# simonhmartin/genomics_general

Measured on AMD Instinct MI355X. Metric: windows_per_sec, higher is better.
Workload: dtype u32 bit-planes / int32 counts / f64 statistics

## Files before the change

genomics_general_amd/csrc/pg_internal.h:

```cpp
#pragma once
#include <hip/hip_runtime.h>
#include <stdint.h>
#include "../../include/popgen_hip.h"
#include "pg_nib.h"

#define PG_MAX_POPS 16
#define PG_SITES_PER_BLOCK 1024
#define PG_ABBA_SITES_PER_BLOCK 4096
#define PG_ABBA_NSUM 6
#define PG_FOURPOP_NSUM 14
#define PG_XV_PLANES 2

#define PG_GROUP 64
#define PG_GROUP_MAX 128
#define PG_XV_CAP(grp) (3 * (grp))
#define PG_XV_CAP_DEFAULT(grp) ((grp) + 1)
#define PG_NP_MAX_SITES 256
#define PG_FLAG_MISMATCH 1
#define PG_FLAG_XV_OVERFLOW 2
#define PG_FLAG_FUSE_STALL 4

struct PgTask2 {
    int32_t row0, nsub, col0, lower;
};

struct PgSynthParams {
    uint64_t seed;
    int64_t first_site_index, scaf_len;
    int32_t n_dip, n_pops, var_thr, miss_thr;
};


void pg_launch_nib_pack(hipStream_t st, const int8_t *src, int S, int n_hap, int64_t n_rows, int8_t *gt, int RS);
void pg_launch_nib_expand(hipStream_t st, const int8_t *gt, int RS, int64_t n_rows, int8_t *dst, int S);
void pg_launch_synth(hipStream_t st, int8_t *gt, int RS, int n_hap, int64_t site0, int64_t n_sites,
                     const int32_t *slot_gen_hap, PgSynthParams p);

void pg_launch_popdist_fin(hipStream_t st, const int32_t *Cmat, const int32_t *Dmat, int N, int cN, int cshift, int n_win,
                           const int32_t *pop_start, int n_pops, int min_pair_sites, double *sum_out,
                           int64_t *cnt_out, int all_diploid, const int64_t *win_lo = nullptr, const int64_t *win_hi = nullptr,
                           long long skip_upto = -1);

void pg_launch_popdist_np(hipStream_t st, const int32_t *Cmat, const int32_t *Dmat, int N, int cN, int cshift, int n_win,
                          const int32_t *pop_start, int n_pops, const int32_t *ref_row, const int32_t *pop_rank,
                          const int32_t *task_tree, const int32_t *trees, int max_leaves, int max_side, int min_pair_sites,
                          double min_data, int do_pairs, double *sums, int64_t *cnts, double *out, const int64_t *win_lo,
                          const int64_t *win_hi, long long max_sites);

void pg_launch_indpair_fin(hipStream_t st, const int32_t *Cmat, const int32_t *Dmat, int N, int cN, int cshift, int n_win,
                           const int32_t *samp_start, const int32_t *samp_rank, int n_samp, int min_pair_sites, double *sum_out,
                           int64_t *cnt_out, int mean_mode);


void pg_launch_abba(hipStream_t st, const int8_t *gt, int RS, const int64_t *win_lo, const int64_t *win_hi,
                    int n_win, int max_chunks, const int32_t *pop_start, int p1, int p2, int p3, int p4,
                    double min_data, int sel, int nsum, double *part_sums, int64_t *part_used, double *sums_out,
                    int64_t *used_out, uint32_t *flags, int64_t base, long long max_sites);

void pg_launch_popfreq(hipStream_t st, const int8_t *gt, int RS, int n_hap, const int64_t *win_lo,
                       const int64_t *win_hi, int n_win, int max_chunks, const int32_t *pop_start, int n_pops,
                       unsigned long long *l_out, unsigned long long *S_out, unsigned long long *pairsum_out,
                       uint32_t *flags, int64_t base);
void pg_launch_popfreq_ordered(hipStream_t st, const int8_t *gt, int RS, const int64_t *win_lo, const int64_t *win_hi, int n_win,
                               const int32_t *pop_start, int n_pops, const uint32_t *flags, int64_t base, double *theta_out);

void pg_launch_site_counts(hipStream_t st, const int8_t *gt, int RS, int64_t site_lo, int64_t site_hi,
                           const int32_t *pop_start, int n_pops, int32_t *cnt_out);
void pg_launch_site_target(hipStream_t st, const int32_t *cnt, int64_t n_sites, int n_pops, int target, double min_data, int as_counts,
                           int has_threshold, double threshold, double *f_out, long long *i_out, uint8_t *keep_out);

void pg_launch_hap_called(hipStream_t st, const int8_t *gt, int RS, int n_hap, const int64_t *win_lo,
                          const int64_t *win_hi, int n_win, int max_chunks, unsigned long long *out);

void pg_launch_pack2(hipStream_t st, const int8_t *gt, int RS, const int64_t *win_lo, const int64_t *win_hi,
                     const int64_t *goff, const int64_t *vgoff, int n_win, int max_groups, int64_t total_groups, uint32_t *Vp,
                     int NPv, uint32_t *XV, int NP, int32_t *nw, int dip, int32_t *mismatch, uint32_t *pres, int capg, int grp);
bool pg_pack_needs_presence(int NP);
struct PgFuseArgs {
    int32_t n_win, kparts, n_units, T, diag;
    int32_t *Cmat;
    signed char a[8][4], b[8][2];
    unsigned char mask[8];
};
bool pg_pack_fuse_fits(int NP, int NPv, int n_units, int n_win);
int pg_launch_pack_fused(hipStream_t st, const int8_t *gt, int RS, const int64_t *win_lo, const int64_t *win_hi, const int64_t *goff,
                         int n_win, int64_t max_words, int64_t avg_words, uint32_t *XV, int NP, int32_t *nw, int dip, int32_t *mismatch,
                         int capg, int n_units, int32_t *Cmat);
void pg_launch_expand(hipStream_t st, const int32_t *Cmat, const int32_t *Dmat, int N, int cN, int cshift, int n_win,
                      int32_t *Cfull, int32_t *Dfull);
void pg_launch_pairC(hipStream_t st, const uint32_t *Vp, const int64_t *vgoff, int n_win, const PgTask2 *tasks, int n_tasks,
                     int NPv, int n_units, int diag, int64_t avg_wq, int32_t *Cmat);
void pg_launch_pairD(hipStream_t st, const uint32_t *XY, const int32_t *nw, const int64_t *goff, int n_win,
                     const PgTask2 *tasks, int n_tasks, int NP, int N, int64_t avg_groups, int32_t *Dmat, int capg);
void pg_launch_pairC_mfma(hipStream_t st, const uint32_t *Vp, const int64_t *vgoff, int n_win, int NPv, int n_units, int diag,
                          int64_t avg_wq, int64_t max_sites, int32_t *Cmat);
void pg_launch_pairD_mfma(hipStream_t st, const uint32_t *XV, const int32_t *nw, const int64_t *goff, int n_win, int NP, int N,
                          int64_t avg_words, int64_t max_vsites, int32_t *Dmat, int capg);

bool pg_pair_tile_fits(int NPv);
int pg_launch_pairC_tile(hipStream_t st, const uint32_t *Vp, const int64_t *vgoff, int n_win, int NPv, int n_units, int diag,
                         int64_t avg_wq, int64_t max_sites, int32_t *Cmat);

bool pg_pair_big_fits(int NPv, int n_units);
void pg_launch_pairC_big(hipStream_t st, const uint32_t *Vp, const int64_t *vgoff, int n_win, int NPv, int n_units, int diag,
                         int64_t avg_wq, int64_t max_sites, int32_t *Cmat);

void pg_launch_sample_het(hipStream_t st, const int32_t *Cmat, const int32_t *Dmat, int N, int cN, int cshift, int n_win,
                          const int32_t *samp_start, int n_samp, int min_pair_sites, double *out);
void pg_launch_hapstats(hipStream_t st, const int32_t *Cmat, const int32_t *Dmat, int N, int cN, int cshift, int n_win,
                        const int32_t *pop_start, int n_pops, int max_pop, const int32_t *order, int min_pair_sites, int diag_nan,
                        double max_dist, uint32_t *bits, size_t bits_per_window, double *out);
void pg_launch_unpack(hipStream_t st, const uint8_t *cells, int n_cols, int64_t n_rows, const int32_t *slot_src, int n_hap,
                      int8_t *gt, int RS);
void pg_launch_flag_export(hipStream_t st, int32_t *flag, double *dst);
void pg_launch_popstats(hipStream_t st, const double *sums, const int64_t *cnts, int n_win, const int32_t *pop_start,
                        int n_pops, double min_data, int do_pairs, double *out, const int64_t *win_lo = nullptr,
                        const int64_t *win_hi = nullptr, long long skip_upto = -1);
```

genomics_general_amd/csrc/pg_pair2.hip:

```cpp
#include "pg_internal.h"

#include <algorithm>
#include <cstdlib>
#include <cstring>

typedef __attribute__((address_space(4))) const uint32_t CU32;

__device__ __forceinline__ void store16(uint32_t *p, uint32_t a, uint32_t b, uint32_t c, uint32_t d) {
    *reinterpret_cast<uint4 *>(p) = make_uint4(a, b, c, d);
}

__device__ __forceinline__ void btrans4(uint32_t t0, uint32_t t1, uint32_t t2, uint32_t t3, uint32_t r[4]) {
    const uint32_t lo01 = __builtin_amdgcn_perm(t1, t0, 0x05010400u), hi01 = __builtin_amdgcn_perm(t1, t0, 0x07030602u);
    const uint32_t lo23 = __builtin_amdgcn_perm(t3, t2, 0x05010400u), hi23 = __builtin_amdgcn_perm(t3, t2, 0x07030602u);
    r[0] = __builtin_amdgcn_perm(lo23, lo01, 0x05040100u);
    r[1] = __builtin_amdgcn_perm(lo23, lo01, 0x07060302u);
    r[2] = __builtin_amdgcn_perm(hi23, hi01, 0x05040100u);
    r[3] = __builtin_amdgcn_perm(hi23, hi01, 0x07060302u);
}

struct RowOff { int v[16]; };

__device__ __forceinline__ RowOff make_row_off(int RS) {
    RowOff ro;
// ... 383 lines not shown
        const uint32_t piece = (a >= q ? (o >> (a - q)) : (o << (q - a))) & (0x11111111u << q);
        pa[a] = q ? (pa[a] | piece) : piece;
    }
}

__device__ __forceinline__ void word_called_presence_keep(const uint32_t d[32], uint32_t v[8], uint32_t pa[4], uint32_t R[4][8]) {
#pragma unroll
    for (int q = 0; q < 4; ++q) {
        uint32_t re[4], ro[4];
        trans_even(d + 8 * q, re);
        trans_odd(d + 8 * q, ro);
        keep_presence(q, re, ro, R[q], pa);
#pragma unroll
        for (int k = 0; k < 8; ++k) {
            const uint32_t t = R[q][k] + 0x77777777u;
            const uint32_t c = (q == 3 ? t : (t >> (3 - q))) & (0x11111111u << q);
            v[k] = q ? (v[k] | c) : c;
        }
    }
}

template <int NWAVE, bool STAGED>
struct XvSink {
    XvWin win;
    int *sh_slot;
    uint4 *cell;
    int stride, burst;
    int nxs;

    __device__ __forceinline__ XvSink(const XvWin &w, int *sh_slot_, uint4 *cell_, int stride_, int burst_)
        : win(w), sh_slot(sh_slot_), cell(cell_), stride(stride_), burst(burst_), nxs(0) {}
    __device__ __forceinline__ void flush() {
        if (!nxs) return;
        const int slot0 = xv_reserve<NWAVE>(win.nwb, nxs, sh_slot);
        for (int k = 0; k < nxs; ++k)
            if (win.template holds<NWAVE>(slot0 + k)) {
                uint4 *o = reinterpret_cast<uint4 *>(win.word(slot0 + k));
#pragma unroll
                for (int i = 0; i < 4; ++i) o[i] = cell[(4 * k + i) * stride];
            }
        nxs = 0;
    }
    __device__ __forceinline__ void put(const uint32_t xo[8], const uint32_t vo[8]) {
        if (STAGED) {
            if (win.has_data) {
#pragma unroll
                for (int i = 0; i < 4; ++i) cell[(4 * nxs + i) * stride] = make_uint4(xo[2 * i], vo[2 * i], xo[2 * i + 1], vo[2 * i + 1]);
            }
            if (++nxs == burst) flush();
        } else {
            const int slot = xv_reserve<NWAVE>(win.nwb, 1, sh_slot);
            if (win.template holds<NWAVE>(slot)) {
                uint32_t *o = win.word(slot);
#pragma unroll
                for (int i = 0; i < 4; ++i) store16(o + 4 * i, xo[2 * i], vo[2 * i], xo[2 * i + 1], vo[2 * i + 1]);
            }
        }
    }
};

__device__ __forceinline__ uint32_t nz_nibbles(uint32_t x) { return ((x + 0x77777777u) >> 3) & 0x11111111u; }


template <class Sink>
struct VsCompactor {
    uint32_t cur[8], xo[8], vo[8];
    int cnt;
    uint32_t MA, ME;
    Sink &out;

    __device__ __forceinline__ explicit VsCompactor(Sink &s) : cnt(0), MA(0u), ME(0u), out(s) {
#pragma unroll
        for (int k = 0; k < 8; ++k) cur[k] = xo[k] = vo[k] = 0u;
    }
    __device__ __forceinline__ void finish_dword(int qd) {
        const uint32_t nME = ~ME;
#pragma unroll
        for (int k = 0; k < 8; ++k) {
            xo[k] |= nz_nibbles(cur[k] & MA) << qd;
            vo[k] |= nz_nibbles(cur[k] & nME) << qd;
            cur[k] = 0u;
        }
        MA = 0u;
        ME = 0u;
    }
    __device__ __forceinline__ void store_word() {
        out.put(xo, vo);
#pragma unroll
        for (int k = 0; k < 8; ++k) xo[k] = vo[k] = 0u;
    }
    __device__ __forceinline__ void append(const uint32_t (&Rq)[8], int j, uint32_t A, uint32_t E) {
        const int sh = 4 * (cnt & 7);
#pragma unroll
        for (int k = 0; k < 8; ++k) cur[k] |= __builtin_amdgcn_ubfe(Rq[k], 4 * j, 4) << sh;
        MA |= A << sh;
        ME |= E << sh;
        ++cnt;
        if ((cnt & 7) == 0) {
            finish_dword((cnt >> 3) - 1);
            if (cnt == 32) {
                store_word();
                cnt = 0;
            }
        }
    }
    __device__ __forceinline__ void finish() {
        if (cnt & 7) finish_dword(cnt >> 3);
        if (cnt) store_word();
    }
};

template <class Sink>
__device__ __forceinline__ void emit_poly_sites(const uint32_t pr[4], const uint32_t (&R)[4][8], VsCompactor<Sink> &vs, int lane) {
    const uint32_t m0 = poly_mask(pr);
    if (m0) {
        const int lb = lane & 31;
        const uint32_t Pl = __builtin_amdgcn_ubfe(pr[0], lb, 1) | (__builtin_amdgcn_ubfe(pr[1], lb, 1) << 1) |
                            (__builtin_amdgcn_ubfe(pr[2], lb, 1) << 2) | (__builtin_amdgcn_ubfe(pr[3], lb, 1) << 3);
        const uint32_t A0l = Pl & (0u - Pl);
#pragma unroll
        for (int q = 0; q < 4; ++q) {
            uint32_t mq = m0 & (0x11111111u << q);
            while (mq) {
                const int bit = __builtin_ctz(mq);
                mq &= mq - 1u;
                vs.append(R[q], bit >> 2, (uint32_t)__builtin_amdgcn_readlane((int)A0l, bit), 0u);
            }
        }
        const uint32_t m3 = tri_mask(pr);
        if (m3) {
#pragma unroll 1
            for (int pass = 1; pass < 3; ++pass) {
                uint32_t m = pass == 1 ? m3 : quad_mask(pr);
                while (m) {
                    const int bit = __builtin_ctz(m);
                    m &= m - 1u;
                    const uint32_t P = (uint32_t)__builtin_amdgcn_readlane((int)Pl, bit);
                    const uint32_t A0 = P & (0u - P), P1 = P ^ A0, A1 = P1 & (0u - P1), P2 = P1 ^ A1, A2 = P2 & (0u - P2);
                    const uint32_t A = pass == 1 ? A1 : A2;
                    const int q = bit & 3;
                    if (q == 0) vs.append(R[0], bit >> 2, A, (A - 1u) & P);
                    else if (q == 1) vs.append(R[1], bit >> 2, A, (A - 1u) & P);
                    else if (q == 2) vs.append(R[2], bit >> 2, A, (A - 1u) & P);
                    else vs.append(R[3], bit >> 2, A, (A - 1u) & P);
                }
            }
        }
    }
}

constexpr int PACK_FUSE_XC = 2;
constexpr int PACK_FUSE_NB = 3;
constexpr int PACK_FUSE_SPINS = 1 << 22;
typedef int fz_v8i __attribute__((ext_vector_type(8)));
typedef float fz_v16f __attribute__((ext_vector_type(16)));

__device__ __forceinline__ fz_v16f fz_mfma(const fz_v8i &a, const fz_v8i &b, const fz_v16f &c) {
    return __builtin_amdgcn_mfma_scale_f32_32x32x64_f8f6f4(a, b, c, 4, 4, 0, 0, 0, 0);
}

__device__ __forceinline__ void fuse_frags(const uint4 *fb, int s, int UW, const int ia[4], const int ib[2], fz_v8i fa_[4], fz_v8i fb_[2]) {
#pragma unroll
    for (int p = 0; p < 4; ++p) {
        const uint4 x = fb[2 * s * UW + ia[p]];
        fa_[p][0] = (int)x.x; fa_[p][1] = (int)x.y; fa_[p][2] = (int)x.z; fa_[p][3] = (int)x.w;
    }
#pragma unroll
    for (int p = 0; p < 2; ++p) {
        const uint4 x = fb[2 * s * UW + ib[p]];
        fb_[p][0] = (int)x.x; fb_[p][1] = (int)x.y; fb_[p][2] = (int)x.z; fb_[p][3] = (int)x.w;
    }
}

__device__ __forceinline__ bool fuse_win_decode(int per_win, int n_win, int &win, int &rem) {
    const int xcd = blockIdx.x & 7;
    const int v = blockIdx.x >> 3;
    const int full = n_win >> 3;
    if (v < full * per_win) {
        win = (v / per_win) * 8 + xcd;
        rem = v % per_win;
        return true;
    }
    const int total = (n_win & 7) * per_win, q = (total + 7) >> 3;
    const int vt = v - full * per_win, lin = xcd * q + vt;
    if (vt >= q || lin >= total) return false;
    win = full * 8 + lin / per_win;
    rem = lin % per_win;
    return true;
}

template <int DIP>
__device__ __forceinline__ void pack3_fused(const int8_t *__restrict__ gt, int RS, const int64_t *__restrict__ win_lo,
                                            const int64_t *__restrict__ win_hi, const int64_t *__restrict__ goff,
                                            uint32_t *__restrict__ XV, int NP, int32_t *__restrict__ nw,
                                            int32_t *__restrict__ mismatch, int capg, const PgFuseArgs &fa) {
    constexpr int VN = DIP ? 4 : 8;
    extern __shared__ uint4 fz_lds[];
    int b, kp;
    if (!fuse_win_decode(fa.kparts, fa.n_win, b, kp)) return;
    const int UW = 32 * fa.T;
    const int lane = threadIdx.x & 63, wave = __builtin_amdgcn_readfirstlane(threadIdx.x >> 6);
    uint4 *const frag = fz_lds;
    uint4 *const stage_x = fz_lds + PACK_FUSE_NB * 8 * UW + wave * (PACK_FUSE_XC * 4 * 64);
    int *const ready = reinterpret_cast<int *>(fz_lds + PACK_FUSE_NB * 8 * UW + 8 * (PACK_FUSE_XC * 4 * 64)), *const done = ready + PACK_FUSE_NB;
    const int64_t lo = win_lo[b], hi = win_hi[b];
    const int W = (int)((hi - lo + 31) >> 5);
    const int w_begin = (int)((long long)W * kp / fa.kparts), w_end = (int)((long long)W * (kp + 1) / fa.kparts);
    const int nit = (w_end - w_begin + 7) >> 3;
    const int h0 = 8 * lane;
    const bool has_data = h0 < 2 * RS;
    const int u0 = VN * lane;
    uint32_t bad = 0u;
    typedef XvSink<1, true> Sink;
    Sink xs(make_xv_win(XV, goff, b, capg, NP, h0, nw, mismatch, has_data), nullptr,  stage_x + lane,  64,
             PACK_FUSE_XC);
    VsCompactor<Sink> vs(xs);
    auto word_rsrc = [&](int w) -> __amdgpu_buffer_rsrc_t {
        const int64_t row = lo + 32ll * w;
        const int n = w < w_end ? (int)((hi - row) < 32 ? (hi - row) : 32) : 0;
        return group_rsrc(gt, RS, n ? row : lo, n);
    };
    const int r = lane & 31, kb = lane >> 5;
    int ia[4], ib[2];
#pragma unroll
    for (int p = 0; p < 4; ++p) ia[p] = kb * UW + 32 * (int)fa.a[wave][p] + r;
#pragma unroll
    for (int p = 0; p < 2; ++p) ib[p] = kb * UW + 32 * (int)fa.b[wave][p] + r;
    fz_v16f acc[4];
#pragma unroll
    for (int p = 0; p < 4; ++p)
#pragma unroll
        for (int e = 0; e < 16; ++e) acc[p][e] = 0.0f;
    if (threadIdx.x < 2 * PACK_FUSE_NB) ready[threadIdx.x] = threadIdx.x == 2 * PACK_FUSE_NB - 1 ? -8 : 0;
    for (int i = threadIdx.x; i < 8 * UW; i += 512) frag[(PACK_FUSE_NB - 1) * 8 * UW + i] = make_uint4(0u, 0u, 0u, 0u);
    bool stalled = false;
    auto wait_ge = [&](int *ctr, int target) {
        for (int spins = 0; __builtin_amdgcn_readfirstlane(__hip_atomic_load(ctr, __ATOMIC_ACQUIRE, __HIP_MEMORY_SCOPE_WORKGROUP)) < target;) {
            __builtin_amdgcn_s_sleep(1);
            if (++spins > PACK_FUSE_SPINS) { stalled = true; break; }
        }
    };
    auto arrive = [&](int *ctr) {
        if (lane == 0) __hip_atomic_fetch_add(ctr, 1, __ATOMIC_RELEASE, __HIP_MEMORY_SCOPE_WORKGROUP);
    };
    uint32_t dn[32];
#pragma unroll
    for (int s = 0; s < 32; ++s) dn[s] = 0u;
    const RowOff ro = make_row_off(RS);
    const int lane_off = has_data ? 4 * lane : 0x40000000;
    word_load(word_rsrc(w_begin + wave), lane_off, RS, 0, ro, dn);
    __syncthreads();
    int slot = 0, round8 = 0, pslot = PACK_FUSE_NB - 1, pround8 = -8;
    for (int it = 0; it < nit; ++it) {
        const int w = w_begin + 8 * it + wave;
        uint32_t pa[4] = {0u, 0u, 0u, 0u};
        uint32_t R[4][8];
        const bool live = w < w_end;
        uint32_t d[32];
#pragma unroll
        for (int s = 0; s < 32; ++s) d[s] = dn[s];
        word_load(word_rsrc(w + 8), lane_off, RS, 0, ro, dn);
        wait_ge(&ready[pslot], pround8 + 8);
        const uint4 *fb = frag + pslot * 8 * UW;
#pragma unroll
        for (int q = 0; q < 4; ++q) {
            fz_v8i fa_[4], fb_[2];
            fuse_frags(fb, q, UW, ia, ib, fa_, fb_);
            uint32_t re[4], rq[4];
            __builtin_amdgcn_sched_barrier(0);
            trans_even(d + 8 * q, re);
            asm volatile("" : "+v"(re[0]), "+v"(re[1]), "+v"(re[2]), "+v"(re[3]));
            __builtin_amdgcn_sched_barrier(0);
            acc[0] = fz_mfma(fa_[0], fb_[0], acc[0]);
            __builtin_amdgcn_sched_barrier(0);
            trans_odd(d + 8 * q, rq);
            asm volatile("" : "+v"(rq[0]), "+v"(rq[1]), "+v"(rq[2]), "+v"(rq[3]));
            __builtin_amdgcn_sched_barrier(0);
            acc[1] = fz_mfma(fa_[1], fb_[1], acc[1]);
            __builtin_amdgcn_sched_barrier(0);
            keep_presence(q, re, rq, R[q], pa);
            asm volatile("" : "+v"(pa[0]), "+v"(pa[1]), "+v"(pa[2]), "+v"(pa[3]));
            __builtin_amdgcn_sched_barrier(0);
            acc[2] = fz_mfma(fa_[2], fb_[0], acc[2]);
            acc[3] = fz_mfma(fa_[3], fb_[1], acc[3]);
            __builtin_amdgcn_sched_barrier(0);
        }
        arrive(&done[pslot]);
        wait_ge(&done[slot], round8);
        {
            uint4 *cell = frag + (slot * 8 + wave) * UW + u0;
#pragma unroll
            for (int k = 0; k < VN; ++k) {
                const int hk = DIP ? 2 * k : k;
                uint32_t c[4];
#pragma unroll
                for (int q = 0; q < 4; ++q) {
                    const uint32_t t = R[q][hk] + 0x77777777u;
                    if (DIP) bad |= t ^ (R[q][hk + 1] + 0x77777777u);
                    c[q] = (t >> 3) & 0x11111111u;
                }
                if (u0 + k < UW) cell[k] = make_uint4(c[0], c[1], c[2], c[3]);
            }
        }
        arrive(&ready[slot]);
        if (live) {
            uint32_t pr[4];
#pragma unroll
            for (int a = 0; a < 4; ++a) pr[a] = pa[a];
            wave_or4(pr);
            emit_poly_sites(pr, R, vs, lane);
        }
        pslot = slot;
        pround8 = round8;
        if (++slot == PACK_FUSE_NB) { slot = 0; round8 += 8; }
    }
    wait_ge(&ready[pslot], pround8 + 8);
#pragma unroll
    for (int q = 0; q < 4; ++q) {
        fz_v8i fa_[4], fb_[2];
        fuse_frags(frag + pslot * 8 * UW, q, UW, ia, ib, fa_, fb_);
#pragma unroll
        for (int p = 0; p < 4; ++p) acc[p] = fz_mfma(fa_[p], fb_[p & 1], acc[p]);
    }
    if (stalled && lane == 0) atomicOr(mismatch, PG_FLAG_FUSE_STALL);
    vs.finish();
    xs.flush();
    if (DIP && (bad & 0x88888888u)) atomicOr(mismatch, 1);
    const int n = fa.n_units, atomic = fa.kparts > 1;
    int32_t *Cw = fa.Cmat + (size_t)b * n * n;
#pragma unroll
    for (int p = 0; p < 4; ++p) {
        if (!((fa.mask[wave] >> p) & 1)) continue;
        const int I = fa.a[wave][p], J = fa.b[wave][p & 1];
        const int col = 32 * J + (lane & 31);
        if (col >= n) continue;
#pragma unroll
        for (int reg = 0; reg < 16; ++reg) {
            const int row = 32 * I + (reg & 3) + 8 * (reg >> 2) + 4 * (lane >> 5);
            if (row >= n || row > col || (row == col && !fa.diag)) continue;
            const int32_t v = (int32_t)(acc[p][reg] * 4.0f);
            int32_t *dst = &Cw[(size_t)row * n + col];
            if (atomic) { if (v) atomicAdd(dst, v); }
            else *dst = v;
        }
    }
}

constexpr int PACK_CELLS = 24;
template <int TPB, int DIP, int BURST, int FUSE>
__global__ __launch_bounds__(TPB) void k_pack3(const int8_t *__restrict__ gt, int RS, const int64_t *__restrict__ win_lo,
                                               const int64_t *__restrict__ win_hi, const int64_t *__restrict__ goff,
                                               const int64_t *__restrict__ vgoff, uint32_t *__restrict__ Vp, int NPv,
                                               uint32_t *__restrict__ XV, int NP, int32_t *__restrict__ nw,
                                               int32_t *__restrict__ mismatch, int capg, int grp, int fq, int perm, PgFuseArgs fa) {
    if constexpr (FUSE) {
        pack3_fused<DIP>(gt, RS, win_lo, win_hi, goff, XV, NP, nw, mismatch, capg, fa);
        return;
    }
    constexpr int NWAVE = TPB / 64;
    constexpr int VN = DIP ? 4 : 8;
    const int FQ = fq, xc = (PACK_CELLS - fq * VN) / 4;
    __shared__ uint32_t sh_pres[2][NWAVE][4];
    __shared__ int sh_slot;
    __shared__ uint4 stage[BURST ? PACK_CELLS * TPB : 1];
    uint4 *const stage_v = stage, *const stage_x = stage + FQ * VN * TPB;
    int nq = 0, wq_first = 0;
    const int b = (int)(((unsigned long long)blockIdx.y * (unsigned)perm) % gridDim.y), g = blockIdx.x;
    const int64_t lo = win_lo[b], hi = win_hi[b];
    const int W = (int)((hi - lo + 31) >> 5);
    const int w_begin = g * grp;
    if (w_begin >= W) return;
    const int w_end = (w_begin + grp < W) ? w_begin + grp : W;
    const int t = threadIdx.x;
    const int lane = threadIdx.x & 63;
    const int h0 = 8 * t;
    const bool has_data = h0 < 2 * RS;
    const int u0 = DIP ? 4 * t : h0;
    const int64_t first = lo + 32ll * w_begin;
    const int nrows = (int)((hi - first) < 32ll * grp ? (hi - first) : 32ll * grp);
    const __amdgpu_buffer_rsrc_t rsrc = group_rsrc(gt, RS, first, nrows);
    int parity = 0;
    uint32_t bad = 0u;
    const int64_t vg_base = vgoff[b] + (int64_t)(w_begin >> 2);
    typedef XvSink<NWAVE, BURST != 0> Sink;
    Sink xs(make_xv_win(XV, goff, b, capg, NP, h0, nw, mismatch, has_data), &sh_slot,  stage_x + t,  TPB,
             xc);
    VsCompactor<Sink> vs(xs);
    auto flush_v = [&]() {
        if (has_data)
            for (int q = 0; q < nq; ++q) {
                uint4 *o = reinterpret_cast<uint4 *>(Vp + ((size_t)(vg_base + wq_first + q) * NPv + u0) * 4u);
#pragma unroll
                for (int k = 0; k < VN; ++k) o[k] = stage_v[(q * VN + k) * TPB + t];
            }
        nq = 0;
    };
    uint32_t dn[32];
#pragma unroll
    for (int s = 0; s < 32; ++s) dn[s] = 0u;
    const RowOff ro = make_row_off(RS);
    if (has_data) word_load(rsrc, 4 * t, RS, 0, ro, dn);
    for (int wq = 0; 4 * wq + w_begin < w_end; ++wq) {
        uint32_t vhold[8][4];
#pragma unroll
        for (int k4 = 0; k4 < 4; ++k4) {
            const int w = w_begin + 4 * wq + k4;
            uint32_t v[8] = {0u, 0u, 0u, 0u, 0u, 0u, 0u, 0u}, pa[4] = {0u, 0u, 0u, 0u};
            uint32_t R[4][8];
#pragma unroll
            for (int q = 0; q < 4; ++q)
#pragma unroll
                for (int k = 0; k < 8; ++k) R[q][k] = 0u;
            const bool live = w < w_end;
            uint32_t d[32];
#pragma unroll
            for (int s = 0; s < 32; ++s) d[s] = dn[s];
            if (has_data) word_load(rsrc, 4 * t, RS, (w + 1 - w_begin) * 32, ro, dn);
            if (live && has_data) word_called_presence_keep(d, v, pa, R);
#pragma unroll
            for (int k = 0; k < 8; ++k) vhold[k][k4] = v[k];
            if (DIP) bad |= (v[0] ^ v[1]) | (v[2] ^ v[3]) | (v[4] ^ v[5]) | (v[6] ^ v[7]);
            if (live) {
                uint32_t pr[4];
#pragma unroll
                for (int a = 0; a < 4; ++a) pr[a] = pa[a];
                block_or4<NWAVE>(pr, sh_pres, parity, lane);
                emit_poly_sites(pr, R, vs, lane);
            }
        }
        if (BURST) {
            if (nq == 0) wq_first = wq;
            if (has_data) {
#pragma unroll
                for (int k = 0; k < VN; ++k) {
                    const int hk = DIP ? 2 * k : k;
                    stage_v[(nq * VN + k) * TPB + t] = make_uint4(vhold[hk][0], vhold[hk][1], vhold[hk][2], vhold[hk][3]);
                }
            }
            if (++nq == FQ) flush_v();
        } else if (has_data) {
            uint32_t *o = Vp + ((size_t)(vg_base + wq) * NPv + u0) * 4u;
#pragma unroll
            for (int k = 0; k < VN; ++k) {
                const int hk = DIP ? 2 * k : k;
                store16(o + 4 * k, vhold[hk][0], vhold[hk][1], vhold[hk][2], vhold[hk][3]);
            }
        }
    }
    vs.finish();
    if (BURST) {
        flush_v();
        xs.flush();
    }
    if (DIP && bad) atomicOr(mismatch, 1);
}

template <int DIP>
static void launch_pack2(hipStream_t st, int threads, dim3 grid, const int8_t *gt, int RS, const int64_t *win_lo,
                         const int64_t *win_hi, const int64_t *goff, const int64_t *vgoff, uint32_t *Vp, int NPv, uint32_t *XV,
                         int NP, int32_t *nw, int32_t *mismatch, uint32_t *pres, int capg, int grp) {
    const bool force2 = getenv("PG_PACK2") != nullptr;
    if (threads <= 1024 && !force2) {
        const int lanes = (threads + 1) / 2;
#define PG_PACK3B(T, B) hipLaunchKernelGGL((k_pack3<T, DIP, B, 0>), grid, dim3(T), 0, st, gt, RS, win_lo, win_hi, goff, vgoff, Vp, NPv, XV, NP, nw, mismatch, capg, grp, fq, perm, PgFuseArgs())
#define PG_PACK3(T) PG_PACK3B(T, 0)
        const int fq = DIP ? 4 : 2;
        int perm = 1;
        if (const char *pe = getenv("PG_PACK_PERM")) {
            const int k = atoi(pe), n = (int)grid.y;
            if (k > 1 && n > 2 * k) {
                auto gcd = [](int a, int b) { while (b) { const int t = a % b; a = b; b = t; } return a; };
                perm = n / k;
                while (gcd(perm, n) != 1) ++perm;
            }
        }
        const bool burst = getenv("PG_PACK_BURST") == nullptr || atoi(getenv("PG_PACK_BURST")) != 0;
        if (lanes <= 64 && burst) PG_PACK3B(64, 1);
        else if (lanes <= 128 && burst) PG_PACK3B(128, 1);
        else if (lanes <= 64) PG_PACK3(64);
        else if (lanes <= 128) PG_PACK3(128);
        else if (lanes <= 256) PG_PACK3(256);
        else PG_PACK3(512);
#undef PG_PACK3
#undef PG_PACK3B
        return;
    }
    if (threads <= 64)
        hipLaunchKernelGGL((k_pack2<64, DIP, 0>), grid, dim3(64), 0, st, gt, RS, win_lo, win_hi, goff, vgoff, Vp, NPv, XV, NP, nw, mismatch, pres, capg, grp);
    else if (threads <= 128)
        hipLaunchKernelGGL((k_pack2<128, DIP, 0>), grid, dim3(128), 0, st, gt, RS, win_lo, win_hi, goff, vgoff, Vp, NPv, XV, NP, nw, mismatch, pres, capg, grp);
    else if (threads <= 256)
        hipLaunchKernelGGL((k_pack2<256, DIP, 0>), grid, dim3(256), 0, st, gt, RS, win_lo, win_hi, goff, vgoff, Vp, NPv, XV, NP, nw, mismatch, pres, capg, grp);
    else {
        grid.z = (threads + 255) / 256;
        hipLaunchKernelGGL(k_presence, grid, dim3(256), 0, st, gt, RS, win_lo, win_hi, goff, pres, grp);
        hipLaunchKernelGGL(k_word_scan, dim3(grid.y), dim3(256), 0, st, win_lo, win_hi, goff, pres, nw, grp);
        hipLaunchKernelGGL((k_pack2<256, DIP, 1>), grid, dim3(256), 0, st, gt, RS, win_lo, win_hi, goff, vgoff, Vp, NPv, XV, NP, nw, mismatch, pres, capg, grp);
    }
}

bool pg_pack_fuse_fits(int NP, int NPv, int n_units, int n_win) {
    const char *f = getenv("PG_PACK_FUSE");
    if (f ? atoi(f) == 0 : (n_win < 1024 || n_units <= 128)) return false;
    for (const char *e : {"PG_PAIR_VALU", "PG_PACK2", "PG_PACK_BURST", "PG_GROUP_WORDS", "PG_PACK_BLOCKS_PER_CU", "PG_OVERLAP", "PG_PACK_PERM"})
        if (getenv(e)) return false;
    return NP <= 512 && n_units >= 1 && pg_pair_big_fits(NPv, n_units);
}

static void pg_fuse_tasks(int T, PgFuseArgs &fa) {
    memset(fa.a, 0, sizeof fa.a);
    memset(fa.b, 0, sizeof fa.b);
    memset(fa.mask, 0, sizeof fa.mask);
    const int Tb = T == 7 ? 6 : T;
    int wv = 0;
    for (int i = 0; i < Tb; i += 2)
        for (int j = i; j < Tb; j += 2, ++wv)
            for (int p = 0; p < 4; ++p) {
                const int I = i + (p >> 1), J = j + (p & 1);
                if (I < Tb && J < Tb && I <= J) {
                    fa.a[wv][p] = (signed char)I;
                    fa.b[wv][p & 1] = (signed char)J;
                    fa.mask[wv] |= (unsigned char)(1u << p);
                }
            }
    if (T == 7)
        for (int i = 0; i < 7; i += 4, ++wv) {
            fa.b[wv][0] = fa.b[wv][1] = 6;
            for (int p = 0; p < 4 && i + p < 7; ++p) {
                fa.a[wv][p] = (signed char)(i + p);
                fa.mask[wv] |= (unsigned char)(1u << p);
            }
        }
}

int pg_launch_pack_fused(hipStream_t st, const int8_t *gt, int RS, const int64_t *win_lo, const int64_t *win_hi, const int64_t *goff,
                         int n_win, int64_t max_words, int64_t avg_words, uint32_t *XV, int NP, int32_t *nw, int dip, int32_t *mismatch,
                         int capg, int n_units, int32_t *Cmat) {
    if (n_win <= 0) return 0;
    PgFuseArgs fa;
    fa.n_win = n_win;
    fa.n_units = n_units;
    fa.T = (n_units + 31) / 32;
    fa.diag = dip ? 1 : 0;
    fa.Cmat = Cmat;
    pg_fuse_tasks(fa.T, fa);
    int64_t kparts = n_win >= 1024 ? 1 : (1024 + n_win - 1) / n_win;
    kparts = std::min<int64_t>(kparts, std::max<int64_t>(1, avg_words / 64));
    kparts = std::max<int64_t>(kparts, (max_words * 32 + (1 << 23) - 1) >> 23);
    fa.kparts = (int)kparts;
    if (kparts > 1) (void)hipMemsetAsync(Cmat, 0, (size_t)n_win * n_units * n_units * 4, st);
    const size_t lds = (size_t)(PACK_FUSE_NB * 8 * 32 * fa.T + 8 * PACK_FUSE_XC * 4 * 64 + 2) * sizeof(uint4);
    const int64_t blocks = (int64_t)((n_win + 7) / 8) * kparts * 8;
#define PG_PACK3F(D)                                                                                                              \
    do {                                                                                                                          \
        static bool ready = false;                                   \
        if (!ready) {                                                                                                             \
            if (hipFuncSetAttribute(reinterpret_cast<const void *>(&k_pack3<512, D, 0, 1>), hipFuncAttributeMaxDynamicSharedMemorySize, \
                                    (PACK_FUSE_NB * 8 * 32 * 7 + 8 * PACK_FUSE_XC * 4 * 64 + 2) * (int)sizeof(uint4)) != hipSuccess) return 1; \
            ready = true;                                                                                                         \
        }                                                                                                                         \
        hipLaunchKernelGGL((k_pack3<512, D, 0, 1>), dim3((unsigned)blocks), dim3(512), lds, st, gt, RS, win_lo, win_hi, goff,         \
                           (const int64_t *)nullptr, (uint32_t *)nullptr, 0, XV, NP, nw, mismatch, capg, 0, 0, 1, fa);           \
    } while (0)
    if (dip) PG_PACK3F(1);
    else PG_PACK3F(0);
#undef PG_PACK3F
    return 0;
}

bool pg_pack_needs_presence(int NP) { return NP / 4 > 1024 || (getenv("PG_PACK2") != nullptr && NP / 4 > 256); }

void pg_launch_pack2(hipStream_t st, const int8_t *gt, int RS, const int64_t *win_lo, const int64_t *win_hi,
                     const int64_t *goff, const int64_t *vgoff, int n_win, int max_groups, int64_t total_groups, uint32_t *Vp,
                     int NPv, uint32_t *XV, int NP, int32_t *nw, int dip, int32_t *mismatch, uint32_t *pres, int capg, int grp) {
    if (n_win <= 0 || max_groups <= 0) return;
    const int threads = NP / 4;
    if (pg_pack_needs_presence(NP)) (void)hipMemsetAsync(pres, 0, (size_t)total_groups * grp * 16u, st);
    dim3 grid(max_groups, n_win);
    if (dip) launch_pack2<1>(st, threads, grid, gt, RS, win_lo, win_hi, goff, vgoff, Vp, NPv, XV, NP, nw, mismatch, pres, capg, grp);
    else launch_pack2<0>(st, threads, grid, gt, RS, win_lo, win_hi, goff, vgoff, Vp, NPv, XV, NP, nw, mismatch, pres, capg, grp);
}

struct PairCtx {
    int win, row0, nsub, col0, lower, lane, ks;
};

__device__ __forceinline__ bool pair_decode(const PgTask2 *__restrict__ tasks, int n_tasks, int kso, int n_win, PairCtx &c) {
    const int xcd = blockIdx.x & 7;
    const int v = blockIdx.x >> 3;
    const int per_win = n_tasks * kso;
    const int full = n_win >> 3;
    int rem;
    if (v < full * per_win) {
        c.win = (v / per_win) * 8 + xcd;
        rem = v % per_win;
    } else {
        const int total = (n_win & 7) * per_win, q = (total + 7) >> 3;
        const int vt = v - full * per_win, lin = xcd * q + vt;
        if (vt >= q || lin >= total) return false;
        c.win = full * 8 + lin / per_win;
        rem = lin % per_win;
    }
    const int wave = __builtin_amdgcn_readfirstlane(threadIdx.x >> 6);
    c.ks = (rem / n_tasks) * 4 + wave;
    c.lane = threadIdx.x & 63;
    const PgTask2 tk = tasks[rem % n_tasks];
    c.row0 = __builtin_amdgcn_readfirstlane(tk.row0);
    c.nsub = __builtin_amdgcn_readfirstlane(tk.nsub);
    c.col0 = __builtin_amdgcn_readfirstlane(tk.col0);
    c.lower = __builtin_amdgcn_readfirstlane(tk.lower);
    return true;
}

template <int R>
__device__ __forceinline__ bool block_reduce(uint32_t (&acc)[R], uint32_t (*red)[64], int lane) {
    const int wave = __builtin_amdgcn_readfirstlane(threadIdx.x >> 6);
    if (wave) {
#pragma unroll
        for (int r = 0; r < R; ++r) red[(wave - 1) * R + r][lane] = acc[r];
    }
    __syncthreads();
    if (wave) return false;
#pragma unroll
    for (int r = 0; r < R; ++r) acc[r] += red[r][lane] + red[R + r][lane] + red[2 * R + r][lane];
    return true;
}

template <int R>
__device__ __forceinline__ void pair_store_circ(const uint32_t (&acc)[R], int row0, int col0, int lane, int nvalid, int n, int diag,
                                                int atomic, int32_t *__restrict__ M) {
    if (lane >= nvalid) return;
    int j = col0 + lane;
    if (j >= n) j -= n;
    const int h = n >> 1;
#pragma unroll
    for (int r = 0; r < R; ++r) {
        const int i = row0 + r;
        if (i >= n) continue;
        int d = j - i;
        if (d < 0) d += n;
        const bool keep = d == 0 ? (diag != 0) : (d <= h && !(2 * d == n && i > j));
        if (!keep) continue;
        int32_t *dst = i <= j ? &M[(size_t)i * n + j] : &M[(size_t)j * n + i];
        if (atomic) { if (acc[r]) atomicAdd(dst, (int32_t)acc[r]); }
        else *dst = (int32_t)acc[r];
    }
}

__device__ __forceinline__ uint32_t bcnt_acc(uint32_t x, uint32_t acc) {
    uint32_t r;
    asm("v_bcnt_u32_b32 %0, %1, %2" : "=v"(r) : "v"(x), "v"(acc));
    return r;
}

#include "pg_pairc_loop.inc"

__device__ __forceinline__ void pairC_body(const uint32_t *__restrict__ Vp, int64_t vg0, int nwq, int NPv, const PairCtx &c,
                                           uint32_t (&acc)[8], int n_units) {
    int j = c.col0 + c.lane;
    if (j >= n_units) j -= n_units;
    const uint32_t stride = (uint32_t)NPv * 16u;
    const int chunk = (int)(0x7fffffffu / stride) > 2 ? (int)(0x7fffffffu / stride) - 2 : 1;
    for (int q0 = 0; q0 < nwq; q0 += chunk) {
        const int nq = (nwq - q0 < chunk) ? nwq - q0 : chunk;
        const uint32_t *base = Vp + (size_t)(vg0 + q0) * NPv * 4u;
        const uint64_t b64 = (uint64_t)base;
        const uint64_t ubase = ((uint64_t)(uint32_t)__builtin_amdgcn_readfirstlane((int)(b64 >> 32)) << 32) |
                               (uint32_t)__builtin_amdgcn_readfirstlane((int)(uint32_t)b64);
        uint32_t soff = (uint32_t)c.row0 * 16u, voff = (uint32_t)j * 16u;
        uint32_t n6 = (uint32_t)__builtin_amdgcn_readfirstlane(nq / 6), rem = (uint32_t)__builtin_amdgcn_readfirstlane(nq % 6);
        asm volatile(PG_PAIRC_LOOP_ASM
                     : "+v"(acc[0]), "+v"(acc[1]), "+v"(acc[2]), "+v"(acc[3]), "+v"(acc[4]), "+v"(acc[5]), "+v"(acc[6]),
                       "+v"(acc[7]), "+s"(soff), "+v"(voff), "+s"(n6)
                     : "s"(ubase), "s"(stride), "s"(rem)
                     : PG_PAIRC_LOOP_CLOBBERS);
    }
}

__global__ __launch_bounds__(256) void k_pairC(const uint32_t *__restrict__ Vp, const int64_t *__restrict__ vgoff, int n_win,
                                               const PgTask2 *__restrict__ tasks, int n_tasks, int kso, int NPv, int n_units,
                                               int diag, int32_t *__restrict__ Cmat) {
    __shared__ uint32_t red[3 * 8][64];
    PairCtx c;
    if (!pair_decode(tasks, n_tasks, kso, n_win, c)) return;
    const int64_t vg_all = vgoff[c.win];
    const int nwq_all = (int)(vgoff[c.win + 1] - vg_all);
    const int parts = 4 * kso;
    const int q0 = (int)((long long)nwq_all * c.ks / parts), q1 = (int)((long long)nwq_all * (c.ks + 1) / parts);
    uint32_t acc[8];
#pragma unroll
    for (int r = 0; r < 8; ++r) acc[r] = 0u;
    if (q1 > q0) pairC_body(Vp, vg_all + q0, q1 - q0, NPv, c, acc, n_units);
    if (block_reduce<8>(acc, red, c.lane)) {
        int32_t *Cw = Cmat + (size_t)c.win * n_units * n_units;
        pair_store_circ<8>(acc, c.row0, c.col0, c.lane, c.nsub, n_units, diag, kso > 1, Cw);
    }
}

static int pick_kso(int n_win, int n_tasks, int64_t steps_per_window, int min_steps) {
    int64_t waves = (int64_t)n_win * n_tasks * 4;
    int ks = 1;
    while (ks < 16 && waves * ks < 8192 && steps_per_window / (ks * 8) >= min_steps) ks *= 2;
    return ks;
}

void pg_launch_pairC(hipStream_t st, const uint32_t *Vp, const int64_t *vgoff, int n_win, const PgTask2 *tasks, int n_tasks,
                     int NPv, int n_units, int diag, int64_t avg_wq, int32_t *Cmat) {
    if (n_win <= 0 || n_tasks <= 0) return;
    const int kso = pick_kso(n_win, n_tasks, avg_wq, 24);
    if (kso > 1) (void)hipMemsetAsync(Cmat, 0, (size_t)n_win * n_units * n_units * 4, st);
    const int64_t blocks = (int64_t)((n_win + 7) / 8) * n_tasks * kso * 8;
    hipLaunchKernelGGL(k_pairC, dim3((unsigned)blocks), dim3(256), 0, st, Vp, vgoff, n_win, tasks, n_tasks, kso, NPv, n_units,
                       diag, Cmat);
}
// ... 78 lines not shown
```

Measured before the change: 344,400.

## Split fused pack kernel into dedicated pack waves and MFMA product waves

Restructures the fused pack+Gram kernel so 8 waves only transpose and pack genotype words into LDS fragments, while 4 additional waves consume those fragments and run the MFMA products. Previously every wave interleaved packing with its share of MFMAs, using host-computed task tables and manual scheduling barriers. The block grows to 768 threads and the producer/consumer handshake moves to ready/done counters. This aims to overlap the integer packing with the matrix work, at the cost of more LDS synchronisation and more accumulators (seven) per product wave, which raises register pressure.

```diff
diff --git a/genomics_general_amd/csrc/pg_internal.h b/genomics_general_amd/csrc/pg_internal.h
--- a/genomics_general_amd/csrc/pg_internal.h
+++ b/genomics_general_amd/csrc/pg_internal.h
@@ -79,8 +79,6 @@
 struct PgFuseArgs {
     int32_t n_win, kparts, n_units, T, diag;
     int32_t *Cmat;
-    signed char a[8][4], b[8][2];
-    unsigned char mask[8];
 };
 bool pg_pack_fuse_fits(int NP, int NPv, int n_units, int n_win);
 int pg_launch_pack_fused(hipStream_t st, const int8_t *gt, int RS, const int64_t *win_lo, const int64_t *win_hi, const int64_t *goff,
diff --git a/genomics_general_amd/csrc/pg_pair2.hip b/genomics_general_amd/csrc/pg_pair2.hip
--- a/genomics_general_amd/csrc/pg_pair2.hip
+++ b/genomics_general_amd/csrc/pg_pair2.hip
@@ -559,6 +559,9 @@
 constexpr int PACK_FUSE_XC = 2;
 constexpr int PACK_FUSE_NB = 3;
 constexpr int PACK_FUSE_SPINS = 1 << 22;
+constexpr int PACK_FUSE_PW = 8;
+constexpr int PACK_FUSE_MW = 4;
+constexpr int PACK_FUSE_TPB = 64 * (PACK_FUSE_PW + PACK_FUSE_MW);
 typedef int fz_v8i __attribute__((ext_vector_type(8)));
 typedef float fz_v16f __attribute__((ext_vector_type(16)));
 
@@ -566,18 +569,25 @@
     return __builtin_amdgcn_mfma_scale_f32_32x32x64_f8f6f4(a, b, c, 4, 4, 0, 0, 0, 0);
 }
 
-__device__ __forceinline__ void fuse_frags(const uint4 *fb, int s, int UW, const int ia[4], const int ib[2], fz_v8i fa_[4], fz_v8i fb_[2]) {
-#pragma unroll
-    for (int p = 0; p < 4; ++p) {
-        const uint4 x = fb[2 * s * UW + ia[p]];
-        fa_[p][0] = (int)x.x; fa_[p][1] = (int)x.y; fa_[p][2] = (int)x.z; fa_[p][3] = (int)x.w;
-    }
-#pragma unroll
-    for (int p = 0; p < 2; ++p) {
-        const uint4 x = fb[2 * s * UW + ib[p]];
-        fb_[p][0] = (int)x.x; fb_[p][1] = (int)x.y; fb_[p][2] = (int)x.z; fb_[p][3] = (int)x.w;
-    }
-}
+__device__ __forceinline__ fz_v8i fuse_frag(const uint4 *cell) {
+    const uint4 x = *cell;
+    fz_v8i f;
+    f[0] = (int)x.x; f[1] = (int)x.y; f[2] = (int)x.z; f[3] = (int)x.w;
+    return f;
+}
+
+struct FuseMeet {
+    bool stalled = false;
+    __device__ __forceinline__ void wait_ge(int *ctr, int target) {
+        for (int spins = 0; __builtin_amdgcn_readfirstlane(__hip_atomic_load(ctr, __ATOMIC_ACQUIRE, __HIP_MEMORY_SCOPE_WORKGROUP)) < target;) {
+            __builtin_amdgcn_s_sleep(1);
+            if (++spins > PACK_FUSE_SPINS) { stalled = true; break; }
+        }
+    }
+    __device__ __forceinline__ void arrive(int *ctr, int lane) {
+        if (lane == 0) __hip_atomic_fetch_add(ctr, 1, __ATOMIC_RELEASE, __HIP_MEMORY_SCOPE_WORKGROUP);
+    }
+};
 
 __device__ __forceinline__ bool fuse_win_decode(int per_win, int n_win, int &win, int &rem) {
     const int xcd = blockIdx.x & 7;
@@ -597,23 +607,11 @@
 }
 
 template <int DIP>
-__device__ __forceinline__ void pack3_fused(const int8_t *__restrict__ gt, int RS, const int64_t *__restrict__ win_lo,
-                                            const int64_t *__restrict__ win_hi, const int64_t *__restrict__ goff,
-                                            uint32_t *__restrict__ XV, int NP, int32_t *__restrict__ nw,
-                                            int32_t *__restrict__ mismatch, int capg, const PgFuseArgs &fa) {
+__device__ __forceinline__ void fuse_pack_wave(const int8_t *__restrict__ gt, int RS, int64_t lo, int64_t hi, int w_begin, int w_end,
+                                               int nit, int b, const int64_t *__restrict__ goff, uint32_t *__restrict__ XV, int NP,
+                                               int32_t *__restrict__ nw, int32_t *__restrict__ mismatch, int capg, int UW, int wave,
+                                               int lane, uint4 *frag, uint4 *stage_x, int *ready, int *done, FuseMeet &meet) {
     constexpr int VN = DIP ? 4 : 8;
-    extern __shared__ uint4 fz_lds[];
-    int b, kp;
-    if (!fuse_win_decode(fa.kparts, fa.n_win, b, kp)) return;
-    const int UW = 32 * fa.T;
-    const int lane = threadIdx.x & 63, wave = __builtin_amdgcn_readfirstlane(threadIdx.x >> 6);
-    uint4 *const frag = fz_lds;
-    uint4 *const stage_x = fz_lds + PACK_FUSE_NB * 8 * UW + wave * (PACK_FUSE_XC * 4 * 64);
-    int *const ready = reinterpret_cast<int *>(fz_lds + PACK_FUSE_NB * 8 * UW + 8 * (PACK_FUSE_XC * 4 * 64)), *const done = ready + PACK_FUSE_NB;
-    const int64_t lo = win_lo[b], hi = win_hi[b];
-    const int W = (int)((hi - lo + 31) >> 5);
-    const int w_begin = (int)((long long)W * kp / fa.kparts), w_end = (int)((long long)W * (kp + 1) / fa.kparts);
-    const int nit = (w_end - w_begin + 7) >> 3;
     const int h0 = 8 * lane;
     const bool has_data = h0 < 2 * RS;
     const int u0 = VN * lane;
@@ -627,75 +625,32 @@
         const int n = w < w_end ? (int)((hi - row) < 32 ? (hi - row) : 32) : 0;
         return group_rsrc(gt, RS, n ? row : lo, n);
     };
-    const int r = lane & 31, kb = lane >> 5;
-    int ia[4], ib[2];
-#pragma unroll
-    for (int p = 0; p < 4; ++p) ia[p] = kb * UW + 32 * (int)fa.a[wave][p] + r;
-#pragma unroll
-    for (int p = 0; p < 2; ++p) ib[p] = kb * UW + 32 * (int)fa.b[wave][p] + r;
-    fz_v16f acc[4];
-#pragma unroll
-    for (int p = 0; p < 4; ++p)
-#pragma unroll
-        for (int e = 0; e < 16; ++e) acc[p][e] = 0.0f;
-    if (threadIdx.x < 2 * PACK_FUSE_NB) ready[threadIdx.x] = threadIdx.x == 2 * PACK_FUSE_NB - 1 ? -8 : 0;
-    for (int i = threadIdx.x; i < 8 * UW; i += 512) frag[(PACK_FUSE_NB - 1) * 8 * UW + i] = make_uint4(0u, 0u, 0u, 0u);
-    bool stalled = false;
-    auto wait_ge = [&](int *ctr, int target) {
-        for (int spins = 0; __builtin_amdgcn_readfirstlane(__hip_atomic_load(ctr, __ATOMIC_ACQUIRE, __HIP_MEMORY_SCOPE_WORKGROUP)) < target;) {
-            __builtin_amdgcn_s_sleep(1);
-            if (++spins > PACK_FUSE_SPINS) { stalled = true; break; }
-        }
-    };
-    auto arrive = [&](int *ctr) {
-        if (lane == 0) __hip_atomic_fetch_add(ctr, 1, __ATOMIC_RELEASE, __HIP_MEMORY_SCOPE_WORKGROUP);
-    };
     uint32_t dn[32];
 #pragma unroll
     for (int s = 0; s < 32; ++s) dn[s] = 0u;
     const RowOff ro = make_row_off(RS);
     const int lane_off = has_data ? 4 * lane : 0x40000000;
     word_load(word_rsrc(w_begin + wave), lane_off, RS, 0, ro, dn);
-    __syncthreads();
-    int slot = 0, round8 = 0, pslot = PACK_FUSE_NB - 1, pround8 = -8;
+    int slot = 0, round = 0;
     for (int it = 0; it < nit; ++it) {
-        const int w = w_begin + 8 * it + wave;
+        const int w = w_begin + PACK_FUSE_PW * it + wave;
         uint32_t pa[4] = {0u, 0u, 0u, 0u};
         uint32_t R[4][8];
         const bool live = w < w_end;
         uint32_t d[32];
 #pragma unroll
         for (int s = 0; s < 32; ++s) d[s] = dn[s];
-        word_load(word_rsrc(w + 8), lane_off, RS, 0, ro, dn);
-        wait_ge(&ready[pslot], pround8 + 8);
-        const uint4 *fb = frag + pslot * 8 * UW;
+        word_load(word_rsrc(w + PACK_FUSE_PW), lane_off, RS, 0, ro, dn);
 #pragma unroll
         for (int q = 0; q < 4; ++q) {
-            fz_v8i fa_[4], fb_[2];
-            fuse_frags(fb, q, UW, ia, ib, fa_, fb_);
             uint32_t re[4], rq[4];
-            __builtin_amdgcn_sched_barrier(0);
             trans_even(d + 8 * q, re);
-            asm volatile("" : "+v"(re[0]), "+v"(re[1]), "+v"(re[2]), "+v"(re[3]));
-            __builtin_amdgcn_sched_barrier(0);
-            acc[0] = fz_mfma(fa_[0], fb_[0], acc[0]);
-            __builtin_amdgcn_sched_barrier(0);
             trans_odd(d + 8 * q, rq);
-            asm volatile("" : "+v"(rq[0]), "+v"(rq[1]), "+v"(rq[2]), "+v"(rq[3]));
-            __builtin_amdgcn_sched_barrier(0);
-            acc[1] = fz_mfma(fa_[1], fb_[1], acc[1]);
-            __builtin_amdgcn_sched_barrier(0);
             keep_presence(q, re, rq, R[q], pa);
-            asm volatile("" : "+v"(pa[0]), "+v"(pa[1]), "+v"(pa[2]), "+v"(pa[3]));
-            __builtin_amdgcn_sched_barrier(0);
-            acc[2] = fz_mfma(fa_[2], fb_[0], acc[2]);
-            acc[3] = fz_mfma(fa_[3], fb_[1], acc[3]);
-            __builtin_amdgcn_sched_barrier(0);
-        }
-        arrive(&done[pslot]);
-        wait_ge(&done[slot], round8);
+        }
+        meet.wait_ge(&done[slot], round);
         {
-            uint4 *cell = frag + (slot * 8 + wave) * UW + u0;
+            uint4 *cell = frag + (slot * PACK_FUSE_PW + wave) * UW + u0;
 #pragma unroll
             for (int k = 0; k < VN; ++k) {
                 const int hk = DIP ? 2 * k : k;
@@ -709,7 +664,7 @@
                 if (u0 + k < UW) cell[k] = make_uint4(c[0], c[1], c[2], c[3]);
             }
         }
-        arrive(&ready[slot]);
+        meet.arrive(&ready[slot], lane);
         if (live) {
             uint32_t pr[4];
 #pragma unroll
@@ -717,40 +672,99 @@
             wave_or4(pr);
             emit_poly_sites(pr, R, vs, lane);
         }
-        pslot = slot;
-        pround8 = round8;
-        if (++slot == PACK_FUSE_NB) { slot = 0; round8 += 8; }
-    }
-    wait_ge(&ready[pslot], pround8 + 8);
-#pragma unroll
-    for (int q = 0; q < 4; ++q) {
-        fz_v8i fa_[4], fb_[2];
-        fuse_frags(frag + pslot * 8 * UW, q, UW, ia, ib, fa_, fb_);
-#pragma unroll
-        for (int p = 0; p < 4; ++p) acc[p] = fz_mfma(fa_[p], fb_[p & 1], acc[p]);
-    }
-    if (stalled && lane == 0) atomicOr(mismatch, PG_FLAG_FUSE_STALL);
+        if (++slot == PACK_FUSE_NB) { slot = 0; round += PACK_FUSE_MW; }
+    }
     vs.finish();
     xs.flush();
     if (DIP && (bad & 0x88888888u)) atomicOr(mismatch, 1);
+}
+
+template <int M, bool FULL>
+__device__ __forceinline__ void fuse_product_wave(const PgFuseArgs &fa, int b, int nit, int UW, int lane, const uint4 *frag,
+                                                  int *ready, int *done, FuseMeet &meet) {
+    const int T = FULL ? 7 : fa.T;
+    const uint4 *const mine = frag + (lane >> 5) * UW + (lane & 31);
+    fz_v16f acc[7];
+#pragma unroll
+    for (int p = 0; p < 7; ++p)
+#pragma unroll
+        for (int e = 0; e < 16; ++e) acc[p][e] = 0.0f;
+    int slot = 0, round = PACK_FUSE_PW;
+    for (int it = 0; it < nit; ++it) {
+        meet.wait_ge(&ready[slot], round);
+        const uint4 *fb = mine + slot * PACK_FUSE_PW * UW;
+#pragma unroll
+        for (int s = 0; s < 4; ++s, fb += 2 * UW) {
+            fz_v8i f[7];
+#pragma unroll
+            for (int j = M; j < 7; ++j) f[j] = fuse_frag(fb + (j < T ? 32 * j : 0));
+#pragma unroll
+            for (int p = 0; p < 7; ++p) {
+                const int I = p < 7 - M ? M : 7 - M, J = p < 7 - M ? M + p : p;
+                if (J < T) acc[p] = fz_mfma(f[I], f[J], acc[p]);
+            }
+        }
+        meet.arrive(&done[slot], lane);
+        if (++slot == PACK_FUSE_NB) { slot = 0; round += PACK_FUSE_PW; }
+    }
     const int n = fa.n_units, atomic = fa.kparts > 1;
     int32_t *Cw = fa.Cmat + (size_t)b * n * n;
 #pragma unroll
-    for (int p = 0; p < 4; ++p) {
-        if (!((fa.mask[wave] >> p) & 1)) continue;
-        const int I = fa.a[wave][p], J = fa.b[wave][p & 1];
-        const int col = 32 * J + (lane & 31);
-        if (col >= n) continue;
+    for (int p = 0; p < 7; ++p) {
+        const int I = p < 7 - M ? M : 7 - M, J = p < 7 - M ? M + p : p;
+        const int c = 32 * J + (lane & 31);
+        if (J >= T || c >= n) continue;
 #pragma unroll
         for (int reg = 0; reg < 16; ++reg) {
-            const int row = 32 * I + (reg & 3) + 8 * (reg >> 2) + 4 * (lane >> 5);
-            if (row >= n || row > col || (row == col && !fa.diag)) continue;
+            const int r = 32 * I + (reg & 3) + 8 * (reg >> 2) + 4 * (lane >> 5);
+            if (r >= n || r > c || (r == c && !fa.diag)) continue;
             const int32_t v = (int32_t)(acc[p][reg] * 4.0f);
-            int32_t *dst = &Cw[(size_t)row * n + col];
+            int32_t *dst = &Cw[(size_t)r * n + c];
             if (atomic) { if (v) atomicAdd(dst, v); }
             else *dst = v;
         }
     }
+}
+
+template <int M>
+__device__ __forceinline__ void fuse_products(const PgFuseArgs &fa, int b, int nit, int UW, int lane, const uint4 *frag, int *ready,
+                                              int *done, FuseMeet &meet) {
+    if (fa.T == 7) fuse_product_wave<M, true>(fa, b, nit, UW, lane, frag, ready, done, meet);
+    else fuse_product_wave<M, false>(fa, b, nit, UW, lane, frag, ready, done, meet);
+}
+
+template <int DIP>
+__device__ __forceinline__ void pack3_fused(const int8_t *__restrict__ gt, int RS, const int64_t *__restrict__ win_lo,
+                                            const int64_t *__restrict__ win_hi, const int64_t *__restrict__ goff,
+                                            uint32_t *__restrict__ XV, int NP, int32_t *__restrict__ nw,
+                                            int32_t *__restrict__ mismatch, int capg, const PgFuseArgs &fa) {
+    extern __shared__ uint4 fz_lds[];
+    int b, kp;
+    if (!fuse_win_decode(fa.kparts, fa.n_win, b, kp)) return;
+    const int UW = 32 * fa.T;
+    const int lane = threadIdx.x & 63, wave = __builtin_amdgcn_readfirstlane(threadIdx.x >> 6);
+    uint4 *const frag = fz_lds;
+    uint4 *const stage = fz_lds + PACK_FUSE_NB * PACK_FUSE_PW * UW;
+    int *const ready = reinterpret_cast<int *>(stage + PACK_FUSE_PW * (PACK_FUSE_XC * 4 * 64)), *const done = ready + PACK_FUSE_NB;
+    if (threadIdx.x < 2 * PACK_FUSE_NB) ready[threadIdx.x] = 0;
+    __syncthreads();
+    const int64_t lo = win_lo[b], hi = win_hi[b];
+    const int W = (int)((hi - lo + 31) >> 5);
+    const int w_begin = (int)((long long)W * kp / fa.kparts), w_end = (int)((long long)W * (kp + 1) / fa.kparts);
+    const int nit = (w_end - w_begin + PACK_FUSE_PW - 1) / PACK_FUSE_PW;
+    FuseMeet meet;
+    if (wave < PACK_FUSE_PW)
+        fuse_pack_wave<DIP>(gt, RS, lo, hi, w_begin, w_end, nit, b, goff, XV, NP, nw, mismatch, capg, UW, wave, lane, frag,
+                            stage + wave * (PACK_FUSE_XC * 4 * 64), ready, done, meet);
+    else {
+        switch (wave - PACK_FUSE_PW) {
+        case 0: fuse_products<0>(fa, b, nit, UW, lane, frag, ready, done, meet); break;
+        case 1: fuse_products<1>(fa, b, nit, UW, lane, frag, ready, done, meet); break;
+        case 2: fuse_products<2>(fa, b, nit, UW, lane, frag, ready, done, meet); break;
+        default: fuse_products<3>(fa, b, nit, UW, lane, frag, ready, done, meet); break;
+        }
+    }
+    if (meet.stalled && lane == 0) atomicOr(mismatch, PG_FLAG_FUSE_STALL);
 }
 
 constexpr int PACK_CELLS = 24;
@@ -914,32 +928,6 @@
     return NP <= 512 && n_units >= 1 && pg_pair_big_fits(NPv, n_units);
 }
 
-static void pg_fuse_tasks(int T, PgFuseArgs &fa) {
-    memset(fa.a, 0, sizeof fa.a);
-    memset(fa.b, 0, sizeof fa.b);
-    memset(fa.mask, 0, sizeof fa.mask);
-    const int Tb = T == 7 ? 6 : T;
-    int wv = 0;
-    for (int i = 0; i < Tb; i += 2)
-        for (int j = i; j < Tb; j += 2, ++wv)
-            for (int p = 0; p < 4; ++p) {
-                const int I = i + (p >> 1), J = j + (p & 1);
-                if (I < Tb && J < Tb && I <= J) {
-                    fa.a[wv][p] = (signed char)I;
-                    fa.b[wv][p & 1] = (signed char)J;
-                    fa.mask[wv] |= (unsigned char)(1u << p);
-                }
-            }
-    if (T == 7)
-        for (int i = 0; i < 7; i += 4, ++wv) {
-            fa.b[wv][0] = fa.b[wv][1] = 6;
-            for (int p = 0; p < 4 && i + p < 7; ++p) {
-                fa.a[wv][p] = (signed char)(i + p);
-                fa.mask[wv] |= (unsigned char)(1u << p);
-            }
-        }
-}
-
 int pg_launch_pack_fused(hipStream_t st, const int8_t *gt, int RS, const int64_t *win_lo, const int64_t *win_hi, const int64_t *goff,
                          int n_win, int64_t max_words, int64_t avg_words, uint32_t *XV, int NP, int32_t *nw, int dip, int32_t *mismatch,
                          int capg, int n_units, int32_t *Cmat) {
@@ -950,23 +938,22 @@
     fa.T = (n_units + 31) / 32;
     fa.diag = dip ? 1 : 0;
     fa.Cmat = Cmat;
-    pg_fuse_tasks(fa.T, fa);
     int64_t kparts = n_win >= 1024 ? 1 : (1024 + n_win - 1) / n_win;
     kparts = std::min<int64_t>(kparts, std::max<int64_t>(1, avg_words / 64));
     kparts = std::max<int64_t>(kparts, (max_words * 32 + (1 << 23) - 1) >> 23);
     fa.kparts = (int)kparts;
     if (kparts > 1) (void)hipMemsetAsync(Cmat, 0, (size_t)n_win * n_units * n_units * 4, st);
-    const size_t lds = (size_t)(PACK_FUSE_NB * 8 * 32 * fa.T + 8 * PACK_FUSE_XC * 4 * 64 + 2) * sizeof(uint4);
+    const size_t lds = (size_t)(PACK_FUSE_NB * PACK_FUSE_PW * 32 * fa.T + PACK_FUSE_PW * PACK_FUSE_XC * 4 * 64 + 2) * sizeof(uint4);
     const int64_t blocks = (int64_t)((n_win + 7) / 8) * kparts * 8;
 #define PG_PACK3F(D)                                                                                                              \
     do {                                                                                                                          \
         static bool ready = false;                                   \
         if (!ready) {                                                                                                             \
-            if (hipFuncSetAttribute(reinterpret_cast<const void *>(&k_pack3<512, D, 0, 1>), hipFuncAttributeMaxDynamicSharedMemorySize, \
-                                    (PACK_FUSE_NB * 8 * 32 * 7 + 8 * PACK_FUSE_XC * 4 * 64 + 2) * (int)sizeof(uint4)) != hipSuccess) return 1; \
+            if (hipFuncSetAttribute(reinterpret_cast<const void *>(&k_pack3<PACK_FUSE_TPB, D, 0, 1>), hipFuncAttributeMaxDynamicSharedMemorySize, \
+                                    (PACK_FUSE_NB * PACK_FUSE_PW * 32 * 7 + PACK_FUSE_PW * PACK_FUSE_XC * 4 * 64 + 2) * (int)sizeof(uint4)) != hipSuccess) return 1; \
             ready = true;                                                                                                         \
         }                                                                                                                         \
-        hipLaunchKernelGGL((k_pack3<512, D, 0, 1>), dim3((unsigned)blocks), dim3(512), lds, st, gt, RS, win_lo, win_hi, goff,         \
+        hipLaunchKernelGGL((k_pack3<PACK_FUSE_TPB, D, 0, 1>), dim3((unsigned)blocks), dim3(PACK_FUSE_TPB), lds, st, gt, RS, win_lo, win_hi, goff,         \
                            (const int64_t *)nullptr, (uint32_t *)nullptr, 0, XV, NP, nw, mismatch, capg, 0, 0, 1, fa);           \
     } while (0)
     if (dip) PG_PACK3F(1);
```

Result: faster. 367,000 (median of 6 runs) (+6.6%).
